# mpi4py/mpi4py-fft

Measured on AMD Instinct MI355X. Metric: pfft_3d_c2c_1024cubed_fp64_gflops, higher is better.
Workload: dtype f64; 1 GPU; PFFT 3D c2c 1024^3 complex128 forward+backward per step

## Files before the change

mpi4py-fft_amd/csrc/fft_fused_f64.hip:

```cpp
#include "fft_fused_impl.h"

namespace gfft {

#ifdef GFFT_VARIANTS
struct Fused1024x8 {
  typedef PassCfg<double, 1024, 16, 8, false, true, PF_NT_LOAD | PF_SYS_STORE | PF_NATURAL, MODE_C2C, false, 16, 16, 4> RowsToRing;
  typedef PassCfg<double, 1024, 16, 8, false, true, PF_NT_STORE | PF_SYS_LOAD | PF_NATURAL, MODE_C2C, false, 16, 16, 4> RowsFromRing;
  typedef PassCfg<double, 1024, 16, 8, true, true, PF_NT_LOAD | PF_C2C_ONLY | PF_SYS_STORE | PF_NATURAL, MODE_C2C, false, 16, 16, 4> ColsToRing;
  typedef PassCfg<double, 1024, 16, 8, true, true, PF_NT_STORE | PF_C2C_ONLY | PF_SYS_LOAD | PF_NATURAL, MODE_C2C, false, 16, 16, 4> ColsFromRing;
  typedef PassCfg<double, 1024, 16, 8, true, true, PF_NT_LOAD | PF_TRANSPOSE_STORE | PF_SYS_STORE | PF_NATURAL, MODE_C2C, true, 16, 16, 4> FourStepFirst;
  typedef PassCfg<double, 1024, 16, 8, true, true, PF_NT_LOAD | PF_SYS_STORE | PF_NATURAL, MODE_C2C, true, 16, 16, 4> FourStepFirstNat;
  typedef PassCfg<double, 1024, 16, 8, false, true, PF_NT_STORE | PF_TRANSPOSE_STORE | PF_SYS_LOAD | PF_NATURAL, MODE_C2C, false, 16, 16, 4> RowsFromRingT;
};
struct Fused1024x8R32 {
  typedef PassCfg<double, 1024, 32, 8, false, true, PF_NT_LOAD | PF_SYS_STORE | PF_NATURAL, MODE_C2C, false, 32, 32> RowsToRing;
  typedef PassCfg<double, 1024, 32, 8, false, true, PF_NT_STORE | PF_SYS_LOAD | PF_NATURAL, MODE_C2C, false, 32, 32> RowsFromRing;
  typedef PassCfg<double, 1024, 32, 8, true, true, PF_NT_LOAD | PF_C2C_ONLY | PF_SYS_STORE | PF_NATURAL, MODE_C2C, false, 32, 32> ColsToRing;
  typedef PassCfg<double, 1024, 32, 8, true, true, PF_NT_STORE | PF_C2C_ONLY | PF_SYS_LOAD | PF_NATURAL, MODE_C2C, false, 32, 32> ColsFromRing;
  typedef PassCfg<double, 1024, 32, 8, true, true, PF_NT_LOAD | PF_TRANSPOSE_STORE | PF_SYS_STORE | PF_NATURAL, MODE_C2C, true, 32, 32> FourStepFirst;
  typedef PassCfg<double, 1024, 32, 8, true, true, PF_NT_LOAD | PF_SYS_STORE | PF_NATURAL, MODE_C2C, true, 32, 32> FourStepFirstNat;
  typedef PassCfg<double, 1024, 32, 8, false, true, PF_NT_STORE | PF_TRANSPOSE_STORE | PF_SYS_LOAD | PF_NATURAL, MODE_C2C, false, 32, 32> RowsFromRingT;
};
#endif

// ... 48 lines not shown
#else
  (void)fuse2_option;
#endif
  if (n_a == n_b && (n_a == 960 || n_a == 896)) {
    if (!g_fuse2_mixv || !cr) return nullptr;
    return n_a == 960 ? fused_pair<Fused960::ColsToRing, Fused960::RowsFromRing>() : fused_pair<Fused896::ColsToRing, Fused896::RowsFromRing>();
  }
  if (n_a == 512 && n_b == 512 && g_fuse2_n512 == 2 && (cr || crb))
    return crb ? fused_pair<Fused512T32::ColsToRingB, Fused512T32::RowsFromRing>() : fused_pair<Fused512T32::ColsToRing, Fused512T32::RowsFromRing>();
  if (n_a != n_b) {
    if (!g_fuse2_mixed || !(cr || crb)) return nullptr;
    if (n_a == 512 && n_b == 1024)
      return crb ? fused_pair<Fused512T32::ColsToRingB, Fused1024R32::RowsFromRing>() : fused_pair<Fused512T32::ColsToRing, Fused1024R32::RowsFromRing>();
    if (n_a == 1024 && n_b == 512)
      return crb ? fused_pair<Fused1024R32::ColsToRingB, Fused512T32::RowsFromRing>() : fused_pair<Fused1024R32::ColsToRing, Fused512T32::RowsFromRing>();
    return nullptr;
  }
  if (n_a != 512 && n_a != 1024) return nullptr;
  if (n_a == 512 && (!g_fuse2_n512 || !(cr || crb || kind == FUSED_PLANES_2D || kind == FUSED_PLANES_2D_B))) return nullptr;
  if (kind == FUSED_PLANES_2D_B)
    return n_a == 512 ? fused_pair<Fused512R32::RowsToRing, Fused512R32::ColsFromRingB>() : fused_pair<Fused1024R32::RowsToRing, Fused1024R32::ColsFromRingB>();
  if (crb)
    return n_a == 512 ? fused_pair<Fused512R32::ColsToRingB, Fused512R32::RowsFromRing>() : fused_pair<Fused1024R32::ColsToRingB, Fused1024R32::RowsFromRing>();
  return n_a == 512 ? pair_of_kind<Fused512R32>(kind) : pair_of_kind<Fused1024R32>(kind);
}

const FusedPair *fused2_select(int precision, int kind, int fuse2_option, int n_a, int n_b) {
  const bool f32 = precision == 4;
  if (fused_kind_real(kind)) return f32 ? fused2_select_real_f32(kind, n_a, n_b) : fused2_select_real_f64(kind, n_a, n_b);
  return f32 ? fused2_select_f32(kind, n_a, n_b) : fused2_select_f64(kind, fuse2_option, n_a, n_b);
}

}
```

mpi4py-fft_amd/csrc/fft_fused_impl.h:

```cpp
#pragma once
#include "fft_pow2_impl.h"

namespace gfft {

template <typename real, int N> struct FusedCfgs;

template <typename A, typename B>
const FusedPair *fused_pair() {
  static const FusedPair p = {&A::ntiles, &B::ntiles, &launch_fused2<A, B>};
  return &p;
}

template <typename C>
static const FusedPair *pair_of_kind(int kind) {
  switch (kind) {
    case FUSED_PLANES_2D:
    case FUSED_ROWS_COLS: return fused_pair<typename C::RowsToRing, typename C::ColsFromRing>();
    case FUSED_COLS_ROWS: return fused_pair<typename C::ColsToRing, typename C::RowsFromRing>();
    case FUSED_FOURSTEP: return fused_pair<typename C::FourStepFirst, typename C::ColsFromRing>();
    case FUSED_FOURSTEP_ROWS: return fused_pair<typename C::FourStepFirstNat, typename C::RowsFromRingT>();
  }
  return nullptr;
}

const FusedPair *fused2_select_f32(int kind, int n_a, int n_b);
const FusedPair *fused2_select_real_f64(int kind, int n_a, int n_b);
const FusedPair *fused2_select_real_f32(int kind, int n_a, int n_b);

}
```

mpi4py-fft_amd/csrc/fft_pow2_impl.h:

```cpp
#pragma once
#include "gfft_internal.h"
#include "pass_io.h"

namespace gfft {

template <typename real> struct K {
  static constexpr real SQ = (real)0.70710678118654752440084436210485;
  static constexpr real C1 = (real)0.92387953251128675612818318939679;
  static constexpr real S1 = (real)0.38268343236508977172845998403040;
};

template <typename real, int S> __device__ __forceinline__ void dft2(cx<real> *v) {
  cx<real> a = v[0], b = v[S];
  v[0] = a + b;
  v[S] = a - b;
}

template <typename real> __device__ __forceinline__ void bf4(cx<real> &a0, cx<real> &a1, cx<real> &a2, cx<real> &a3) {
  cx<real> t0 = a0 + a2, t1 = a0 - a2, t2 = a1 + a3, t3 = mul_mi(a1 - a3);
  a0 = t0 + t2;
  a1 = t1 + t3;
  a2 = t0 - t2;
  a3 = t1 - t3;
}
// ... 1026 lines not shown
          }
        }
      }
    }
  }
  __syncthreads();
}

#ifdef GFFT_FUSE2_TRACE
#define GFFT_TRACE_SLOTS 96
#define GFFT_TRACE_STAMP(i)                                                                                    \
  if (it < GFFT_TRACE_SLOTS && wave_of_thread0()) {                                                              \
    if (threadIdx.x == 0) trace[((size_t)blockIdx.x * GFFT_TRACE_SLOTS + it) * 16 + (i)] = wall_clock64();      \
  }
#else
#define GFFT_TRACE_STAMP(i)
#endif

template <typename A, typename B> constexpr int fused2_per_cu() {
  constexpr size_t lds = A::lds > B::lds ? A::lds : B::lds;
  constexpr int budget = (A::regs_per_thread >= 64 || B::regs_per_thread >= 64) ? 256 : 128;
  return (2 * A::threads / 256 * budget <= 512 && 2 * lds + 1024 <= 160 * 1024) ? 2 : 1;
}
template <typename A, typename B>
__global__ void __launch_bounds__(A::threads, (fused2_per_cu<A, B>() * A::threads / 256))
fft_fused2_kernel(const PassDesc *__restrict__ descs, FusedDesc f, double scale_a, double scale_b, const void *__restrict__ in,
                  void *__restrict__ ring, void *__restrict__ out) {
  static_assert(A::threads == B::threads, "both passes of a fused pair run on one workgroup shape");
  const PassDesc &dA = descs[0], &dB = descs[1];
  extern __shared__ __attribute__((aligned(16))) unsigned char smem[];
  __shared__ unsigned tk[4];
  unsigned *done_a = f.ctr + 16, *done_b = f.ctr + 16 + f.planes;
  const unsigned grp = (unsigned)f.group;
  const unsigned ta = (unsigned)f.tiles_a / grp, tb = (unsigned)f.tiles_b / grp, per_pair = ta + tb;
  const unsigned head = (unsigned)f.lag * ta, pairs = (unsigned)(f.planes - f.lag);
  const unsigned total = (unsigned)f.planes * per_pair;
#ifdef GFFT_FUSE2_TRACE
  unsigned long long *trace = reinterpret_cast<unsigned long long *>(f.ctr + ((16 + 2 * (size_t)f.planes + 63) & ~(size_t)63));
  unsigned it = 0;
#endif
  if (wave_of_thread0()) {
    if (threadIdx.x == 0) tk[0] = atomicAdd(&f.ctr[0], 1u);
  }
  int owed = -1;
  auto settle = [&]() {
    if (owed >= 0) {
      __builtin_amdgcn_s_waitcnt(0);
      __syncthreads();
      if (wave_of_thread0()) {
        if (threadIdx.x == 0) __hip_atomic_fetch_add(&done_a[owed], 1u, __ATOMIC_RELAXED, __HIP_MEMORY_SCOPE_AGENT);
      }
      owed = -1;
    }
  };
  auto await = [&](const unsigned *flag, unsigned want) {
    if (owed >= 0) {
      if (wave_of_thread0()) {
        if (threadIdx.x == 0) tk[2] = __hip_atomic_load(flag, __ATOMIC_RELAXED, __HIP_MEMORY_SCOPE_AGENT) >= want ? 1u : 0u;
      }
// ... 7 lines not shown
#ifdef GFFT_FUSE2_TRACE
  auto hook = [&]() {
    settle();
    __builtin_amdgcn_s_waitcnt(0);
    GFFT_TRACE_STAMP(2)
  };
  for (it = 0;; ++it) {
#else
  auto &hook = settle;
  for (unsigned it = 0;; ++it) {
#endif
#ifdef GFFT_FUSE2_TRACE
    if (wave_of_thread0()) {
      if (threadIdx.x == 0) gfft_trace_slot = it < GFFT_TRACE_SLOTS ? trace + ((size_t)blockIdx.x * GFFT_TRACE_SLOTS + it) * 16 : nullptr;
    }
#endif
    __syncthreads();
    const unsigned k = __builtin_amdgcn_readfirstlane(tk[it & 1]);
    if (k >= total) break;
    GFFT_TRACE_STAMP(0)
    if (wave_of_thread0()) {
      if (threadIdx.x == 0) tk[(it + 1) & 1] = atomicAdd(&f.ctr[0], 1u);
    }
    bool is_a;
    unsigned p, t;
    if (k < head) {
      is_a = true; p = k / ta; t = k - p * ta;
    } else {
      const unsigned k2 = k - head;
      if (k2 < pairs * per_pair) {
        const unsigned j = k2 / per_pair, r = k2 - j * per_pair;
        if (r < tb) { is_a = false; p = j; t = r; } else { is_a = true; p = j + (unsigned)f.lag; t = r - tb; }
      } else {
        const unsigned k3 = k2 - pairs * per_pair, j = k3 / tb;
        is_a = false; p = pairs + j; t = k3 - j * tb;
      }
    }
    char *slot = static_cast<char *>(ring) + (size_t)(p % (unsigned)f.ring) * f.slot_bytes;
    if (f.debug == 2) continue;
#ifdef GFFT_FUSE2_TRACE
    if (it < GFFT_TRACE_SLOTS && wave_of_thread0()) {
      if (threadIdx.x == 0) trace[((size_t)blockIdx.x * GFFT_TRACE_SLOTS + it) * 16 + 7] = ((unsigned long long)k << 1) | (is_a ? 1u : 0u);
    }
#endif
    if (is_a) {
      if (p >= (unsigned)f.ring) await(&done_b[p - f.ring], tb);
      else if (f.defer == 2) settle();
      GFFT_TRACE_STAMP(1)
      if (f.debug != 3 && f.debug != 5)
        for (unsigned g = 0; g < grp; ++g)
          A::tile(dA, static_cast<const char *>(in) + (size_t)p * f.a_in_plane, slot, smem, t * grp + g, scale_a, hook);
      GFFT_TRACE_STAMP(3)
      owed = (int)p;
      if (!f.defer) settle();
      GFFT_TRACE_STAMP(4)
    } else {
      await(&done_a[p], ta);
      GFFT_TRACE_STAMP(1)
      if (f.debug != 3 && f.debug != 4)
        for (unsigned g = 0; g < grp; ++g)
          B::tile(dB, slot, static_cast<char *>(out) + (size_t)p * f.b_out_plane, smem, t * grp + g, scale_b, hook);
      GFFT_TRACE_STAMP(3)
      __syncthreads();
      if (wave_of_thread0()) {
        if (threadIdx.x == 0) __hip_atomic_fetch_add(&done_b[p], 1u, __ATOMIC_RELAXED, __HIP_MEMORY_SCOPE_AGENT);
      }
      GFFT_TRACE_STAMP(4)
    }
  }
  settle();
}


template <typename A, typename B>
hipError_t launch_fused2(const PassDesc &dA, const PassDesc &dB, const PassDesc *dev_descs, const FusedDesc &f, const void *in,
                         void *ring, void *out, hipStream_t s) {
  constexpr size_t lds = A::lds > B::lds ? A::lds : B::lds;
  static_assert(lds <= 160 * 1024, "LDS budget");
  if (f.lag < 1 || f.ring <= f.lag || f.planes < 1 || f.tiles_a != (int)A::ntiles(dA) || f.tiles_b != (int)B::ntiles(dB) ||
      f.group < 1 || f.tiles_a % f.group || f.tiles_b % f.group)
    return hipErrorInvalidValue;
  auto kern = fft_fused2_kernel<A, B>;
  static bool attr_set[kMaxDevices] = {};
  static int cus_of[kMaxDevices] = {};
  const int dev = current_device();
  if (!attr_set[dev] && lds > 64 * 1024) {
    hipError_t e = hipFuncSetAttribute(reinterpret_cast<const void *>(kern), hipFuncAttributeMaxDynamicSharedMemorySize, (int)lds);
    if (e != hipSuccess) return e;
    attr_set[dev] = true;
  }
  if (!cus_of[dev]) {
    int n = 0;
    if (hipDeviceGetAttribute(&n, hipDeviceAttributeMultiprocessorCount, dev) != hipSuccess || n < 1) { (void)hipGetLastError(); n = 256; }
    cus_of[dev] = n;
  }
  const int cus = cus_of[dev];
  hipError_t e = hipMemsetAsync(f.ctr, 0, (size_t)(16 + 2 * f.planes) * sizeof(unsigned), s);
  if (e != hipSuccess) return e;
  constexpr int per_cu = fused2_per_cu<A, B>();
  hipLaunchKernelGGL(kern, dim3(cus * per_cu), dim3(A::threads), lds, s, dev_descs, f, dA.scale, dB.scale, in, ring, out);
  return hipGetLastError();
}


template <typename real, int N, int R, int T, bool COLS, bool SPLIT, int MINW, int FLAGS, int MODE, bool BIGTW, int... RADS>
// ... 134 lines not shown
```

mpi4py-fft_amd/csrc/gfft_internal.h:

```cpp
#pragma once
#include <hip/hip_runtime.h>
#include <stdint.h>
#include <string>

namespace gfft {

int fail(int code, const std::string &msg);
int hip_fail(hipError_t e, const char *what);
int check_device();
int scratch_get(hipStream_t s, size_t bytes, void **out);
#define HIP_TRY(expr)                                        \
  do {                                                       \
    hipError_t _e = (expr);                                  \
    if (_e != hipSuccess) return gfft::hip_fail(_e, #expr);  \
  } while (0)

constexpr int kMaxDevices = 64;
inline int current_device() {
  int d = 0;
  if (hipGetDevice(&d) != hipSuccess) { (void)hipGetLastError(); d = 0; }
  return (d < 0 || d >= kMaxDevices) ? 0 : d;
}

template <typename T> struct cx { T x, y; };

template <typename T> __device__ __forceinline__ cx<T> operator+(cx<T> a, cx<T> b) { return {a.x + b.x, a.y + b.y}; }
// ... 87 lines not shown

inline bool strided_lines_whole(const PassDesc &d, int esz) {
  auto ok = [&](int64_t s) { return (s * esz) % 128 == 0; };
  if (!ok(d.in_es) || !ok(d.out_es)) return false;
  const int64_t rows = d.mid * d.inner > 0 ? d.batch / (d.mid * d.inner) : 1;
  if (d.mid > 1 && !d.flat && (!ok(d.in_ms) || !ok(d.out_ms))) return false;
  if (rows > 1 && (!ok(d.in_os) || !ok(d.out_os))) return false;
  if ((d.in_lgp && !ok(d.in_jump)) || (d.out_lgp && !ok(d.out_jump))) return false;
  return true;
}

bool pow2_supported_f64(int n);
bool pow2_supported_f32(int n);
hipError_t launch_pow2_f64(const PassDesc &d, bool cols, int variant, const void *in, void *out, hipStream_t s);
hipError_t launch_pow2_f32(const PassDesc &d, bool cols, int variant, const void *in, void *out, hipStream_t s);
bool pow2_r2r_supported(int n);
hipError_t launch_pow2_r2r_f64(const PassDesc &d, bool cols, const void *in, void *out, hipStream_t s);
hipError_t launch_pow2_r2r_f32(const PassDesc &d, bool cols, const void *in, void *out, hipStream_t s);
int pow2_grid_cap();
struct FusedDesc {
  int planes, tiles_a, tiles_b, ring, lag;
  int defer;
  int group;
  int64_t a_in_plane, b_out_plane;
  int64_t slot_bytes;
  unsigned debug;
  unsigned wait_ticks;
  unsigned plan_id;
  unsigned *host_flag;
  unsigned *ctr;
};
enum FusedKind { FUSED_ROWS_COLS = 0, FUSED_COLS_ROWS = 1, FUSED_FOURSTEP = 2, FUSED_PLANES_2D = 3, FUSED_FOURSTEP_ROWS = 4,
                 FUSED_R2C_PLANES = 5, FUSED_COLS_C2R = 6,
                 FUSED_PLANES_2D_B = 7, FUSED_PLANES_CR_B = 8,
                 FUSED_R2C_PLANES_B = 9, FUSED_COLS_C2R_B = 10 };
struct FusedKindInfo { const char *pass_name, *describe_name; bool real; };
inline constexpr FusedKindInfo kFusedKinds[] = {
  {"fused rows+cols", "rows -> strided", false},
  {"fused cols+rows", "strided -> rows", false},
  {"fused four-step", "four-step", false},
  {"fused 2-D rows+cols", "2-D planes: rows -> strided", false},
  {"fused four-step (rows)", "four-step: strided -> rows, transposed on store", false},
  {"fused r2c-rows+cols", "r2c rows -> strided", true},
  {"fused cols+c2r-rows", "strided -> c2r rows", true},
  {"fused 2-D rows+cols(blocks)", "2-D planes: rows -> strided into blocks", false},
  {"fused 2-D cols(blocks)+rows", "2-D planes: strided from blocks -> rows", false},
  {"fused 2-D r2c-rows+cols(blocks)", "2-D planes: r2c rows -> strided into blocks", true},
  {"fused 2-D cols(blocks)+c2r-rows", "2-D planes: strided from blocks -> c2r rows", true},
};
static_assert(sizeof kFusedKinds / sizeof kFusedKinds[0] == FUSED_COLS_C2R_B + 1, "one row per FusedKind");
inline bool fused_kind_real(int kind) { return kFusedKinds[kind].real; }
extern int g_fuse2_n512;
extern int g_fuse2_mixed;
extern int g_fuse2_f32_n512;
extern int g_fuse2_mixv;
extern int g_c2r_2048;
struct FusedPair {
  unsigned (*tiles_a)(const PassDesc &), (*tiles_b)(const PassDesc &);
  hipError_t (*launch)(const PassDesc &dA, const PassDesc &dB, const PassDesc *dev_descs, const FusedDesc &f, const void *in,
                       void *ring, void *out, hipStream_t s);
};
const FusedPair *fused2_select(int precision, int kind, int fuse2_option, int n_a, int n_b);

bool real_half_supported(int n_complex);
hipError_t launch_real_half_f64(const PassDesc &d, int variant, const void *in, void *out, hipStream_t s);
hipError_t launch_real_half_f32(const PassDesc &d, int variant, const void *in, void *out, hipStream_t s);
bool real_half_mix_supported(int n_complex);
hipError_t launch_real_half_mix_f64(const PassDesc &d, const void *in, void *out, hipStream_t s);
hipError_t launch_real_half_mix_f32(const PassDesc &d, const void *in, void *out, hipStream_t s);
bool mix3_supported(int n);
hipError_t launch_mix3_f64(const PassDesc &d, bool cols, const void *in, void *out, hipStream_t s);
hipError_t launch_mix3_f32(const PassDesc &d, bool cols, const void *in, void *out, hipStream_t s);
bool mixv_supported(int n);
hipError_t launch_mixv_f64(const PassDesc &d, bool cols, int variant, const void *in, void *out, hipStream_t s);
hipError_t launch_mixv_f32(const PassDesc &d, bool cols, int variant, const void *in, void *out, hipStream_t s);
hipError_t launch_real_half_mixv_f64(const PassDesc &d, const void *in, void *out, hipStream_t s);
hipError_t launch_real_half_mixv_f32(const PassDesc &d, const void *in, void *out, hipStream_t s);
bool mix5_supported(int n);
hipError_t launch_mix5_f64(const PassDesc &d, bool cols, const void *in, void *out, hipStream_t s);
hipError_t launch_mix5_f32(const PassDesc &d, bool cols, const void *in, void *out, hipStream_t s);

bool plane2d_supported(int n, int precision);
int plane2d_pitch(int n);
// ... 19 lines not shown
```

mpi4py-fft_amd/csrc/plan.cpp:

```cpp
#include "../../include/gfft.h"
#include "gfft_internal.h"

#include <atomic>
#include <cmath>
#include <cstdio>
#include <cstdlib>
#include <cstring>
#include <map>
#include <tuple>
#include <mutex>
#include <string>
#include <thread>
#include <vector>

using namespace gfft;

namespace {

thread_local std::string g_last_error;
bool g_device_checked = false;

}

namespace gfft {
// ... 23 lines not shown
}

namespace {

struct Options {
  int grid_cap = 0;
  int variant_rows = 0;
  int variant_cols = 0;
  int force_generic = 0;
  int xcd_swizzle = -1;
  int tile_order = -1;
  int profile = 0;
  int fused3 = 1;
  int debug_flat = 0;
  int flat_out = 1;
  int mixv_variant = 0;
  int mixv = 1;
  int wtile = 1;
  int plane2d = 1;
  int fuse2 = 1;
  int fuse2_ring = 0, fuse2_lag = 0;
  int fuse2_kinds = 2046;
  int fuse2_f32 = 1;
  int fuse2_wait_ms = 2000;
  int debug_tile_lg = 0, debug_tile_side = 0, debug_tile_stride = 0;
  int64_t fused3_min_bytes = 32 << 20;
  int debug_tw_index = 1, debug_tw_exp = 0, debug_tw_len = 0;
  int debug_r2r_index = 1, debug_r2r_exp = 0, debug_r2r_post = 0;
  Options() {
    if (const char *s = getenv("GFFT_GRID_CAP")) grid_cap = atoi(s);
    if (const char *s = getenv("GFFT_VARIANT_ROWS")) variant_rows = atoi(s);
    if (const char *s = getenv("GFFT_VARIANT_COLS")) variant_cols = atoi(s);
    if (const char *s = getenv("GFFT_FORCE_GENERIC")) force_generic = atoi(s);
    if (const char *s = getenv("GFFT_FUSED3")) fused3 = atoi(s);
    if (const char *s = getenv("GFFT_XCD_SWIZZLE")) xcd_swizzle = atoi(s);
    if (const char *s = getenv("GFFT_FUSE2")) fuse2 = atoi(s);
    if (const char *s = getenv("GFFT_FUSE2_RING")) fuse2_ring = atoi(s);
    if (const char *s = getenv("GFFT_FUSE2_LAG")) fuse2_lag = atoi(s);
    if (const char *s = getenv("GFFT_FUSE2_KINDS")) fuse2_kinds = atoi(s);
    if (const char *s = getenv("GFFT_FUSE2_WAIT_MS")) fuse2_wait_ms = atoi(s);
  }
};
Options &opts() {
  static Options o;
  return o;
}

int dev_prec(int precision) { return precision + (current_device() << 8); }
std::mutex g_tw_mutex;
std::map<std::tuple<int64_t, int, int>, void *> g_tw_cache;
struct BigTw { void *hi, *lo; int L; };
std::map<std::pair<int64_t, int>, BigTw> g_bigtw_cache;

int upload_twiddles(int64_t n, int64_t step, int64_t count, int precision, void **out, int64_t wrong_index = -1, double wrong_by = 0) {
  const long double w = -2.0L * 3.14159265358979323846264338327950288L / (long double)n;
  std::vector<unsigned char> host((size_t)count * 2 * precision);
  for (int64_t j = 0; j < count; ++j) {
    const int64_t k = (j * step) % n;
    long double c, s;
    {
      const long double a = w * (long double)k;
      c = cosl(a);
      s = sinl(a);
// ... 67 lines not shown
  bool regk = false, cols = false;
  int src = BUF_IN, dst = BUF_OUT;
  bool carries_scale = false;
  bool logical_first = false;
  PointDesc pt{};
  double extra_scale = 1.0;
  bool has_full = false;
  PassDesc full{};
  int64_t data_inner = 0;
  int blocks[2] = {1, 1};
  int64_t bstride[2] = {0, 0};
  PassDesc d2{};
  FusedDesc fused{};
  int fused_kind = 0;
  const FusedPair *pair = nullptr;
  PassDesc *dev_descs = nullptr;
  int alt_first = -1;
  int alt_buf = -1;
  size_t alt_bytes = 0;
  double bytes2 = 0;
};

bool make_fused2(gfft_plan_s *pl, int kind, const Pass &a, const Pass &b, const PassDesc &dA, const PassDesc &dB, int planes,
                 int64_t a_in_plane, int64_t b_out_plane, int64_t slot_bytes, Pass *out);

bool is_pow2(int64_t n) { return n > 0 && (n & (n - 1)) == 0; }

static int pow2_rows_nt(int64_t n, int precision) {
  if (!is_pow2(n) || n < 16 || n > 4096) return 0;
  if (n <= 32) return 4;
  if (n == 64) return 8;
  if (n == 128) return 16;
  if (n == 256) return precision == 8 ? 32 : 16;
  if (n <= 1024) return 64;
  return (int)(n / 16);
}

bool regk_ok(int64_t n, int precision) {
  if (opts().force_generic) return false;
  if (n > 4096) return false;
  if (mix3_supported((int)n) || mix5_supported((int)n)) return true;
  return precision == 8 ? pow2_supported_f64((int)n) : pow2_supported_f32((int)n);
}

bool regk_c2c_ok(int64_t n, int precision, int mode) {
  (void)precision;
  return !opts().force_generic && opts().mixv && mode == MODE_C2C && n <= 4096 && mixv_supported((int)n);
// ... 257 lines not shown
    if (hipGetDeviceProperties(&prop, dev) == hipSuccess) {
      if (!strncmp(prop.gcnArchName, "gfx942", 6) || !strncmp(prop.gcnArchName, "gfx950", 6)) arch_ok[dev] = 1;
    } else {
      (void)hipGetLastError();
    }
  }
  return arch_ok[dev] > 0;
}

struct PairChoice {
  const FusedPair *pair = nullptr;
  int ring = 0, lag = 0;
};
PairChoice fused2_pair(int precision, int kind, int n_a, int n_b, int64_t slot_bytes, int planes) {
  PairChoice c;
  if (!fused2_arch_ok()) return c;
  if (!opts().fuse2 || !((opts().fuse2_kinds >> kind) & 1)) return c;
  if (precision == GFFT_F32 && (!opts().fuse2_f32 || (fused_kind_real(kind) && opts().fuse2_f32 < 2))) return c;
  if (!fused2_ring(precision, n_a, n_b, slot_bytes, planes, &c.ring, &c.lag)) return c;
  c.pair = fused2_select(precision, kind, opts().fuse2, n_a, n_b);
  return c;
}

bool make_fused2(gfft_plan_s *pl, int kind, const Pass &a, const Pass &b, const PassDesc &dA, const PassDesc &dB, int planes,
                 int64_t a_in_plane, int64_t b_out_plane, int64_t slot_bytes, Pass *out) {
  const PairChoice c = fused2_pair(pl->precision, kind, dA.n, dB.n, slot_bytes, planes);
  if (!c.pair) return false;
  const int ta = (int)c.pair->tiles_a(dA), tb = (int)c.pair->tiles_b(dB);
  if (ta < 1 || tb < 1) return false;
  if (slot_bytes >= ((int64_t)1 << 31) || (double)planes * (ta + tb) >= 1.0e9) return false;
  Pass f = a;
  f.kind = PK_FUSED2;
  f.fused_kind = kind;
  f.pair = c.pair;
  f.d = dA;
  f.d2 = dB;
  f.src = a.src;
  f.dst = b.dst;
  f.carries_scale = false;
  f.fused.planes = planes;
  f.fused.tiles_a = ta;
  f.fused.tiles_b = tb;
  f.fused.ring = c.ring;
  f.fused.lag = c.lag;
  f.fused.defer = 0;
  f.fused.group = 1;
  f.fused.a_in_plane = a_in_plane;
  f.fused.b_out_plane = b_out_plane;
  f.fused.slot_bytes = (int64_t)align256((size_t)slot_bytes);
  f.fused.ctr = nullptr;
  f.fused.wait_ticks = 0;
  f.fused.plan_id = pl->id;
  f.fused.host_flag = nullptr;
  f.fused.debug = 0;
  for (const Pass *q : {&a, &b})
    for (int side : {q->src, q->dst})
      if (side >= BUF_WS && side != BUF_RING) f.alt_buf = side;

  size_t ctr_bytes = align256((size_t)(16 + 2 * planes) * sizeof(unsigned));
#ifdef GFFT_FUSE2_TRACE
  ctr_bytes += 256 + (size_t)1024 * 96 * 16 * sizeof(unsigned long long);
#endif
  const PassDesc both[2] = {f.d, f.d2};
  void *dev = nullptr;
  if (hipMalloc(&dev, sizeof both) != hipSuccess) { (void)hipGetLastError(); return false; }
  if (hipMemcpy(dev, both, sizeof both, hipMemcpyHostToDevice) != hipSuccess) { (void)hipGetLastError(); (void)hipFree(dev); return false; }
  pl->device_allocs.push_back(dev);
  f.dev_descs = static_cast<PassDesc *>(dev);
  need(pl, BUF_RING, (size_t)c.ring * (size_t)f.fused.slot_bytes + ctr_bytes);
  f.alt_first = (int)pl->alt.size();
  pl->alt.push_back(a);
  pl->alt.push_back(b);
  *out = f;
  return true;
}

struct Line {
  int64_t outer, inner, n, nin, nout;
  int mode;
  bool inverse;
  int src, dst;
};

int plan_line(gfft_plan_s *pl, const Line &L, bool top);

PassDesc natural_desc(const Line &L) {
  PassDesc d{};
  d.n = (int)L.n;
  d.mode = L.mode;
  d.conj_in = L.inverse ? 1 : 0;
  d.conj_out = (L.inverse && L.mode != MODE_C2R) ? 1 : 0;
  d.batch = L.outer * L.inner;
// ... 689 lines not shown
    seq.push_back(axis0_flat(BUF_WS, BUF_OUT));
  } else if (!inverse && !cols_first) {
    seq.push_back(rows(real ? MODE_R2C : MODE_C2C, false, true, BUF_IN, BUF_WS));
    seq.push_back(axis0(BUF_WS, BUF_WS));
    seq.push_back(axis1(true, false, BUF_WS, BUF_OUT));
  } else {
    seq.push_back(axis1(false, true, BUF_IN, BUF_WS));
    seq.push_back(axis0(BUF_WS, BUF_WS));
    seq.push_back(rows(real ? MODE_C2R : MODE_C2C, true, false, BUF_WS, BUF_OUT));
  }
  for (Pass &p : seq) {
    int rc = get_twiddles(p.d.n, prec, &p.d.tw);
    if (rc) return rc;
    const bool half = p.d.mode == MODE_R2C_H || p.d.mode == MODE_C2R_H;
    if (half && (rc = get_twiddles(2 * (int64_t)p.d.n, prec, &p.d.rtw))) return rc;
    const double lines = p.data_inner ? (double)p.d.batch / (double)p.d.inner * (double)p.data_inner : (double)p.d.batch;
    const double n = half ? 2.0 * p.d.n : p.d.n;
    pl->flops += (p.d.mode == MODE_C2C ? 1.0 : 0.5) * 5.0 * n * std::log2(n) * lines;
    pl->bytes += fused3_pass_bytes(p, prec, nc_full);
    pl->passes.push_back(p);
  }
  auto fuse = [&](size_t i, int kind, const PassDesc &dA, const PassDesc &dB, int64_t planes, int64_t a_in_plane, int64_t b_out_plane, int64_t slot_bytes) {
    Pass f;
    if (!make_fused2(pl, kind, pl->passes[i], pl->passes[i + 1], dA, dB, (int)planes, a_in_plane, b_out_plane, slot_bytes, &f)) return;
    f.bytes2 = fused3_pass_bytes(pl->passes[i], prec, nc_full) + fused3_pass_bytes(pl->passes[i + 1], prec, nc_full);
    pl->passes[i] = f;
    pl->passes.erase(pl->passes.begin() + i + 1);
  };
  if (!real && !tr && !flat_out && Pu == nc && pl->passes.size() >= 3) {
    const size_t base = pl->passes.size() - 3;
    const Pass &p1 = pl->passes[base], &p2 = pl->passes[base + 1], &p3 = pl->passes[base + 2];
    if (!inverse && !cols_first) {
      PassDesc dA = p1.d, dB = p2.d;
      dA.batch = n0; dA.inner = 1; dA.in_is = 0; dA.out_is = 0; dA.out_os = P;
      dB.batch = Pu; dB.in_os = 0; dB.out_os = 0; dB.in_es = P;
      fuse(base, FUSED_ROWS_COLS, dA, dB, n1, n2 * esz, w_i1 * esz, n0 * P * esz);
    } else {
      PassDesc dA = p2.d, dB = p3.d;
      dA.batch = Pu; dA.in_os = 0; dA.out_os = 0; dA.out_es = P;
      dB.batch = n0; dB.inner = 1; dB.in_is = 0; dB.out_is = 0; dB.in_os = P; dB.out_os = n1 * n2;
      int64_t a_plane = w_i1 * esz;
      if (wtile) {
        dA.mid = Pu / TWc; dA.inner = TWc;
        dA.in_ms = wtS; dA.in_is = 1; dA.in_ilg = 0; dA.in_iS = 0;
        dA.out_ms = TWc;     dA.out_is = 1; dA.out_ilg = 0; dA.out_iS = 0;
        dB.in_tlg = 0; dB.in_tS = 0;
        a_plane = TWc * esz;
// ... 281 lines not shown
}

int gfft_device_name(int device, char *buf, size_t len) {
  hipDeviceProp_t prop;
  HIP_TRY(hipGetDeviceProperties(&prop, device));
  snprintf(buf, len, "%s (%s, %d CUs)", prop.name, prop.gcnArchName, prop.multiProcessorCount);
  return GFFT_OK;
}

int gfft_set_option(const char *key, int value) {
  if (!key) return fail(GFFT_ERR_INVALID, "null option name");
  if (!strcmp(key, "grid_cap")) opts().grid_cap = value;
  else if (!strcmp(key, "variant_rows")) opts().variant_rows = value;
  else if (!strcmp(key, "variant_cols")) opts().variant_cols = value;
  else if (!strcmp(key, "force_generic")) opts().force_generic = value;
  else if (!strcmp(key, "copy_nt")) gfft::g_copy_nt = value;
  else if (!strcmp(key, "fused3")) opts().fused3 = value;
  else if (!strcmp(key, "plane2d")) opts().plane2d = value;
  else if (!strcmp(key, "fuse2")) opts().fuse2 = value;
  else if (!strcmp(key, "fuse2_ring")) opts().fuse2_ring = value;
  else if (!strcmp(key, "fuse2_lag")) opts().fuse2_lag = value;
  else if (!strcmp(key, "fuse2_kinds")) opts().fuse2_kinds = value;
  else if (!strcmp(key, "fuse2_wait_ms")) opts().fuse2_wait_ms = value;
  else if (!strcmp(key, "fuse2_f32")) opts().fuse2_f32 = value;
  else if (!strcmp(key, "fuse2_n512")) gfft::g_fuse2_n512 = value;
  else if (!strcmp(key, "c2r_2048")) gfft::g_c2r_2048 = value;
  else if (!strcmp(key, "fuse2_mixv")) gfft::g_fuse2_mixv = value;
  else if (!strcmp(key, "fuse2_mixed")) gfft::g_fuse2_mixed = value;
  else if (!strcmp(key, "fuse2_f32_n512")) gfft::g_fuse2_f32_n512 = value;
  else if (!strcmp(key, "debug_flat")) opts().debug_flat = value;
  else if (!strcmp(key, "flat_out")) opts().flat_out = value;
  else if (!strcmp(key, "wtile")) opts().wtile = value;
  else if (!strcmp(key, "mixv")) opts().mixv = value;
  else if (!strcmp(key, "mixv_variant")) opts().mixv_variant = value;
  else if (!strcmp(key, "debug_tile_lg")) opts().debug_tile_lg = value;
  else if (!strcmp(key, "debug_tile_side")) opts().debug_tile_side = value;
  else if (!strcmp(key, "debug_tile_stride")) opts().debug_tile_stride = value;
  else if (!strcmp(key, "profile")) opts().profile = value;
  else if (!strcmp(key, "debug_tw_index")) opts().debug_tw_index = value;
  else if (!strcmp(key, "debug_tw_exp")) opts().debug_tw_exp = value;
  else if (!strcmp(key, "debug_tw_len")) opts().debug_tw_len = value;
  else if (!strcmp(key, "debug_r2r_index")) opts().debug_r2r_index = value;
  else if (!strcmp(key, "debug_r2r_exp")) opts().debug_r2r_exp = value;
  else if (!strcmp(key, "debug_r2r_post")) opts().debug_r2r_post = value;
  else if (!strcmp(key, "xcd_swizzle")) opts().xcd_swizzle = value;
  else if (!strcmp(key, "tile_order")) opts().tile_order = value;
// ... 287 lines not shown
        const Pass &q = pl->alt[p.alt_first + k];
        PassDesc dq = q.d;
        const bool sc = k == 1 && p.carries_scale;
        if (sc) dq.scale = scale;
        HIP_TRY(run_pass(pl, q, dq, bufs[q.src], bufs[q.dst], sc ? scale : 1.0, s));
      }
      HIP_TRY(mark());
      continue;
    }
    if (p.kind == PK_FUSED2) {
      PassDesc d2 = p.d2;
      if (p.carries_scale) d2.scale = scale;
      FusedDesc f = p.fused;
      char *ring = static_cast<char *>(bufs[BUF_RING]);
      f.ctr = reinterpret_cast<unsigned *>(ring + (size_t)f.ring * (size_t)f.slot_bytes);
      {
        AsyncErrors &ae = async_errors();
        f.host_flag = (ae.flag && pl->async_slot >= 0) ? ae.flag + pl->async_slot : nullptr;
        const int ms = opts().fuse2_wait_ms;
        f.wait_ticks = ms <= 0 ? 0u : (ms > 40000 ? 4000000000u : (unsigned)ms * 100000u);
      }
      static const int debug = getenv("GFFT_FUSE2_DEBUG") ? atoi(getenv("GFFT_FUSE2_DEBUG")) : 0;
      if (debug) { f.wait_ticks = 100000u; f.host_flag = nullptr; f.debug = (unsigned)debug; }
      HIP_TRY(p.pair->launch(d, d2, p.dev_descs, f, bufs[p.src], ring, bufs[p.dst], s));
      if (debug) {
        HIP_TRY(hipStreamSynchronize(s));
        std::vector<unsigned> h(16 + 2 * (size_t)f.planes);
        HIP_TRY(hipMemcpy(h.data(), f.ctr, h.size() * sizeof(unsigned), hipMemcpyDeviceToHost));
        unsigned long long sa = 0, sb = 0;
        for (int i = 0; i < f.planes; ++i) { sa += h[16 + i]; sb += h[16 + f.planes + i]; }
        fprintf(stderr, "[gfft fuse2] kind %d planes %d tiles %d+%d ring %d lag %d: tickets %u, waits given up %u, A tiles %llu, B tiles %llu\n",
                p.fused_kind, f.planes, f.tiles_a, f.tiles_b, f.ring, f.lag, h[0], h[1], sa, sb);
#ifdef GFFT_FUSE2_TRACE
        if (const char *path = getenv("GFFT_FUSE2_TRACE_FILE")) {
          std::vector<unsigned long long> tr((size_t)1024 * 96 * 16);
          const size_t off = ((16 + 2 * (size_t)f.planes + 63) & ~(size_t)63) * sizeof(unsigned);
          HIP_TRY(hipMemcpy(tr.data(), reinterpret_cast<char *>(f.ctr) + off, tr.size() * sizeof(tr[0]), hipMemcpyDeviceToHost));
          if (FILE *fp = fopen(path, "wb")) { fwrite(tr.data(), sizeof(tr[0]), tr.size(), fp); fclose(fp); }
        }
#endif
      }
      HIP_TRY(mark());
      continue;
    }
    if (p.carries_scale) d.scale = scale;
    HIP_TRY(run_pass(pl, p, d, bufs[p.src], bufs[p.dst], p.carries_scale ? scale : 1.0, s));
    HIP_TRY(mark());
// ... 428 lines not shown
  d.ub_tlg = lg;
  for (int b = 0; b < 8; ++b) d.ub_base[b] = b < nblocks ? d.ub_rows * (int64_t)d.ub_start[b] : 0;
  return GFFT_OK;
}

int gfft_scratch_release(void) { return scratch_pool().release(true); }

int gfft_async_error(void) { return poll_async_error(nullptr); }
int gfft_plan_status(gfft_plan pl) {
  if (!pl) return fail(GFFT_ERR_INVALID, "null plan");
  return poll_async_error(pl);
}

int gfft_plan_destroy(gfft_plan pl) {
  if (!pl) return GFFT_OK;
  delete pl;
  if (--g_live_plans == 0) (void)scratch_pool().release(false);
  return GFFT_OK;
}

int gfft_plan_describe(gfft_plan pl, char *buf, size_t len) {
  if (!pl || !buf || !len) return fail(GFFT_ERR_INVALID, "null argument");
  std::string s;
  char line[256];
  const char *kn = pl->kind == GFFT_C2C_FORWARD ? "c2c-forward" : pl->kind == GFFT_C2C_BACKWARD ? "c2c-backward"
                   : pl->kind == GFFT_R2C ? "r2c" : "c2r";
  char sched[96] = "";
  if (pl->fused3 && pl->ws_tile) snprintf(sched, sizeof sched, " [3-D schedule: tile-major workspace, tiles of %d columns]", pl->ws_tile);
  else if (pl->fused3) snprintf(sched, sizeof sched, " [3-D schedule: padded-pitch workspace, rows %lld entries apart]", (long long)pl->ws_pitch);
  snprintf(line, sizeof line, "gfft plan: %s %s, %d dims, %zu passes%s\n", kn, pl->precision == 8 ? "f64" : "f32",
           pl->ndims, pl->passes.size(), sched);
  s += line;
  static const char *bufn[] = {"IN", "OUT", "WS", "FS", "AUX", "RING", "FS2"};
  for (const Pass &p : pl->passes) {
    if (p.kind == PK_FUSED2) {
      const char *fk = kFusedKinds[p.fused_kind].describe_name;
      if (pl->fused_off)
        snprintf(line, sizeof line, "  pair (%s) n=%d then n=%d as two stand-alone passes (a fused launch gave up a wait)%s  %s -> %s\n",
                 fk, p.d.n, p.d2.n, p.carries_scale ? " [scale]" : "", bufn[p.src], bufn[p.dst]);
      else
      snprintf(line, sizeof line, "  fused pair (%s) n=%d then n=%d: %d planes, %d + %d tiles per plane, ring of %d slots x %lld KiB, one persistent launch%s  %s -> %s\n",
               fk, p.d.n, p.d2.n, p.fused.planes, p.fused.tiles_a, p.fused.tiles_b, p.fused.ring,
               (long long)(p.fused.slot_bytes >> 10), p.carries_scale ? " [scale]" : "", bufn[p.src], bufn[p.dst]);
      s += line;
      continue;
    }
    if (p.kind == PK_PLANE2D) {
      snprintf(line, sizeof line, "  planes on chip: rows n=%d then columns n=%d of %d planes held in LDS, one launch%s  %s -> %s\n", p.d.n, p.d2.n,
               p.fused.planes, p.carries_scale ? " [scale]" : "", bufn[p.src], bufn[p.dst]);
      s += line;
      continue;
    }
    if (p.kind != PK_FFT) {
      static const char *kinds[] = {"", "embed (chirp/zero-pad into AUX)", "multiply by B = FFT(chirp)", "extract (chirp, scale)"};
      snprintf(line, sizeof line, "  %s n=%lld Lw=%lld  %s -> %s\n", kinds[p.kind], (long long)p.pt.n,
               (long long)p.pt.Lw, bufn[p.src], bufn[p.dst]);
      s += line;
      continue;
    }
    snprintf(line, sizeof line, "  n=%d batch=%lld (mid=%lld inner=%lld) es_in=%lld es_out=%lld kernel=%s%s%s  %s -> %s\n",
             p.d.n, (long long)p.d.batch, (long long)p.d.mid, (long long)p.d.inner, (long long)p.d.in_es,
             (long long)p.d.out_es,
             (p.d.mode == MODE_R2C_H || p.d.mode == MODE_C2R_H) ? "regs-rows packed-real (n = complex length)"
             : p.regk ? (p.cols ? "regs-cols" : "regs-rows") : "generic",
             p.d.tw_hi ? " [four-step 1/2, fused twiddle]" : "", p.carries_scale ? " [scale]" : "",
             bufn[p.src], bufn[p.dst]);
// ... 145 lines not shown
```

Before: 10570 GFLOP/s.

## Add paired-plane ticket order for fused 1024 cols-rows persistent kernel

Adds a second ticket-to-work mapping for the persistent fused two-pass kernel. Planes are interleaved in pairs spaced d apart, and the ring size and lag are re-planned so the ring gap constraints still hold. It is enabled by default for the f64 1024x1024 cols-rows pair under the 3-D schedule. The goal is to change the order in which stage-A and stage-B tiles are processed, which affects locality and how long workers wait on plane dependencies. In exchange it may enlarge the ring buffer (up to 256 MiB) and adds extra index arithmetic per ticket.

```diff
diff --git a/mpi4py-fft_amd/csrc/fft_fused_f64.hip b/mpi4py-fft_amd/csrc/fft_fused_f64.hip
--- a/mpi4py-fft_amd/csrc/fft_fused_f64.hip
+++ b/mpi4py-fft_amd/csrc/fft_fused_f64.hip
@@ -94,6 +94,7 @@
     return n_a == 512 ? fused_pair<Fused512R32::RowsToRing, Fused512R32::ColsFromRingB>() : fused_pair<Fused1024R32::RowsToRing, Fused1024R32::ColsFromRingB>();
   if (crb)
     return n_a == 512 ? fused_pair<Fused512R32::ColsToRingB, Fused512R32::RowsFromRing>() : fused_pair<Fused1024R32::ColsToRingB, Fused1024R32::RowsFromRing>();
+  if (cr && n_a == 1024) return fused_pair<Fused1024R32::ColsToRing, Fused1024R32::RowsFromRing, true>();
   return n_a == 512 ? pair_of_kind<Fused512R32>(kind) : pair_of_kind<Fused1024R32>(kind);
 }
 
diff --git a/mpi4py-fft_amd/csrc/fft_fused_impl.h b/mpi4py-fft_amd/csrc/fft_fused_impl.h
--- a/mpi4py-fft_amd/csrc/fft_fused_impl.h
+++ b/mpi4py-fft_amd/csrc/fft_fused_impl.h
@@ -5,10 +5,15 @@
 
 template <typename real, int N> struct FusedCfgs;
 
-template <typename A, typename B>
+template <typename A, typename B, bool WITH_PAIR_ORDER = false>
 const FusedPair *fused_pair() {
-  static const FusedPair p = {&A::ntiles, &B::ntiles, &launch_fused2<A, B>};
-  return &p;
+  if constexpr (WITH_PAIR_ORDER) {
+    static const FusedPair p = {&A::ntiles, &B::ntiles, &launch_fused2<A, B>, &launch_fused2<A, B, true>};
+    return &p;
+  } else {
+    static const FusedPair p = {&A::ntiles, &B::ntiles, &launch_fused2<A, B>, nullptr};
+    return &p;
+  }
 }
 
 template <typename C>
diff --git a/mpi4py-fft_amd/csrc/fft_pow2_impl.h b/mpi4py-fft_amd/csrc/fft_pow2_impl.h
--- a/mpi4py-fft_amd/csrc/fft_pow2_impl.h
+++ b/mpi4py-fft_amd/csrc/fft_pow2_impl.h
@@ -1072,7 +1072,7 @@
   constexpr int budget = (A::regs_per_thread >= 64 || B::regs_per_thread >= 64) ? 256 : 128;
   return (2 * A::threads / 256 * budget <= 512 && 2 * lds + 1024 <= 160 * 1024) ? 2 : 1;
 }
-template <typename A, typename B>
+template <typename A, typename B, bool PAIR_ORDER = false>
 __global__ void __launch_bounds__(A::threads, (fused2_per_cu<A, B>() * A::threads / 256))
 fft_fused2_kernel(const PassDesc *__restrict__ descs, FusedDesc f, double scale_a, double scale_b, const void *__restrict__ in,
                   void *__restrict__ ring, void *__restrict__ out) {
@@ -1082,9 +1082,8 @@
   __shared__ unsigned tk[4];
   unsigned *done_a = f.ctr + 16, *done_b = f.ctr + 16 + f.planes;
   const unsigned grp = (unsigned)f.group;
-  const unsigned ta = (unsigned)f.tiles_a / grp, tb = (unsigned)f.tiles_b / grp, per_pair = ta + tb;
-  const unsigned head = (unsigned)f.lag * ta, pairs = (unsigned)(f.planes - f.lag);
-  const unsigned total = (unsigned)f.planes * per_pair;
+  const unsigned ta = (unsigned)f.tiles_a / grp, tb = (unsigned)f.tiles_b / grp;
+  const unsigned total = (unsigned)f.planes * (ta + tb);
 #ifdef GFFT_FUSE2_TRACE
   unsigned long long *trace = reinterpret_cast<unsigned long long *>(f.ctr + ((16 + 2 * (size_t)f.planes + 63) & ~(size_t)63));
   unsigned it = 0;
@@ -1138,20 +1137,13 @@
     if (wave_of_thread0()) {
       if (threadIdx.x == 0) tk[(it + 1) & 1] = atomicAdd(&f.ctr[0], 1u);
     }
-    bool is_a;
-    unsigned p, t;
-    if (k < head) {
-      is_a = true; p = k / ta; t = k - p * ta;
-    } else {
-      const unsigned k2 = k - head;
-      if (k2 < pairs * per_pair) {
-        const unsigned j = k2 / per_pair, r = k2 - j * per_pair;
-        if (r < tb) { is_a = false; p = j; t = r; } else { is_a = true; p = j + (unsigned)f.lag; t = r - tb; }
-      } else {
-        const unsigned k3 = k2 - pairs * per_pair, j = k3 / tb;
-        is_a = false; p = pairs + j; t = k3 - j * tb;
-      }
-    }
+    FusedTicket tkt;
+    if constexpr (PAIR_ORDER)
+      tkt = fused_ticket(k, ta, tb, (unsigned)f.planes, (unsigned)f.lag >> 1, fused_order_upair((unsigned)f.planes, (unsigned)f.d), (unsigned)f.d);
+    else
+      tkt = fused_ticket_plain(k, ta, tb, (unsigned)f.planes, (unsigned)f.lag);
+    const bool is_a = tkt.is_a;
+    const unsigned p = tkt.plane, t = tkt.tile;
     char *slot = static_cast<char *>(ring) + (size_t)(p % (unsigned)f.ring) * f.slot_bytes;
     if (f.debug == 2) continue;
 #ifdef GFFT_FUSE2_TRACE
@@ -1188,7 +1180,7 @@
 }
 
 
-template <typename A, typename B>
+template <typename A, typename B, bool PAIR_ORDER = false>
 hipError_t launch_fused2(const PassDesc &dA, const PassDesc &dB, const PassDesc *dev_descs, const FusedDesc &f, const void *in,
                          void *ring, void *out, hipStream_t s) {
   constexpr size_t lds = A::lds > B::lds ? A::lds : B::lds;
@@ -1196,7 +1188,8 @@
   if (f.lag < 1 || f.ring <= f.lag || f.planes < 1 || f.tiles_a != (int)A::ntiles(dA) || f.tiles_b != (int)B::ntiles(dB) ||
       f.group < 1 || f.tiles_a % f.group || f.tiles_b % f.group)
     return hipErrorInvalidValue;
-  auto kern = fft_fused2_kernel<A, B>;
+  if ((f.order != 0) != PAIR_ORDER || (f.order && ((f.lag & 1) || !fused_order_fits(f.planes, f.ring, f.lag / 2, f.d)))) return hipErrorInvalidValue;
+  auto kern = fft_fused2_kernel<A, B, PAIR_ORDER>;
   static bool attr_set[kMaxDevices] = {};
   static int cus_of[kMaxDevices] = {};
   const int dev = current_device();
diff --git a/mpi4py-fft_amd/csrc/fused_order.h b/mpi4py-fft_amd/csrc/fused_order.h
--- /dev/null
+++ b/mpi4py-fft_amd/csrc/fused_order.h
@@ -0,0 +1,113 @@
+#pragma once
+
+#if defined(__HIPCC__)
+#define GFFT_HD __host__ __device__ __forceinline__
+#else
+#define GFFT_HD inline
+#endif
+
+namespace gfft {
+
+struct FusedTicket {
+  bool is_a;
+  unsigned plane, tile;
+};
+
+GFFT_HD FusedTicket fused_ticket_plain(unsigned k, unsigned ta, unsigned tb, unsigned planes, unsigned lag) {
+  FusedTicket t;
+  const unsigned per_pair = ta + tb, head = lag * ta, pairs = planes - lag;
+  if (k < head) {
+    t.is_a = true; t.plane = k / ta; t.tile = k - t.plane * ta;
+  } else {
+    const unsigned k2 = k - head;
+    if (k2 < pairs * per_pair) {
+      const unsigned j = k2 / per_pair, r = k2 - j * per_pair;
+      if (r < tb) { t.is_a = false; t.plane = j; t.tile = r; } else { t.is_a = true; t.plane = j + lag; t.tile = r - tb; }
+    } else {
+      const unsigned k3 = k2 - pairs * per_pair, j = k3 / tb;
+      t.is_a = false; t.plane = pairs + j; t.tile = k3 - j * tb;
+    }
+  }
+  return t;
+}
+
+GFFT_HD unsigned fused_order_upair(unsigned planes, unsigned d) { return d ? (planes / (2u * d)) * d : 0u; }
+GFFT_HD unsigned fused_order_unit(unsigned p, unsigned upair, unsigned d) {
+  return p < 2u * upair ? (p / (2u * d)) * d + (p % (2u * d)) % d : p - upair;
+}
+
+GFFT_HD void fused_order_locate(unsigned x, unsigned n, unsigned v0, unsigned upair, unsigned d, unsigned &plane, unsigned &tile) {
+  const unsigned in_pairs = v0 < upair ? (upair - v0) * 2u * n : 0u;
+  if (x < in_pairs) {
+    const unsigned v = v0 + x / (2u * n), r = x % (2u * n);
+    plane = (v / d) * 2u * d + v % d + (r & 1u) * d;
+    tile = r >> 1;
+  } else {
+    x -= in_pairs;
+    plane = (v0 > upair ? v0 : upair) + upair + x / n;
+    tile = x % n;
+  }
+}
+
+GFFT_HD FusedTicket fused_ticket(unsigned k, unsigned ta, unsigned tb, unsigned planes, unsigned lead, unsigned upair, unsigned d) {
+  FusedTicket t;
+  const unsigned head = (lead + (lead < upair ? lead : upair)) * ta;
+  if (k < head) {
+    t.is_a = true;
+    fused_order_locate(k, ta, 0u, upair, d, t.plane, t.tile);
+    return t;
+  }
+  k -= head;
+  const unsigned jm = planes - upair - lead;
+  const unsigned j1 = upair > lead ? upair - lead : 0u;
+  const unsigned j2 = upair < jm ? upair : jm;
+  unsigned j0 = 0u, nj = j1, sb = 2u * tb, sa = 2u * ta;
+  if (k >= nj * (sa + sb)) {
+    k -= nj * (sa + sb);
+    j0 = j1; nj = j2 - j1; sa = ta;
+    if (k >= nj * (sa + sb)) {
+      k -= nj * (sa + sb);
+      j0 = j2; nj = jm - j2; sb = tb;
+      if (k >= nj * (sa + sb)) {
+        k -= nj * (sa + sb);
+        t.is_a = false;
+        fused_order_locate(k, tb, jm, upair, d, t.plane, t.tile);
+        return t;
+      }
+    }
+  }
+  const unsigned j = j0 + k / (sa + sb), r = k % (sa + sb);
+  t.is_a = r >= sb;
+  if (t.is_a) fused_order_locate(r - sb, ta, j + lead, upair, d, t.plane, t.tile);
+  else fused_order_locate(r, tb, j, upair, d, t.plane, t.tile);
+  return t;
+}
+
+inline int fused_order_gap(int planes, int ring, int d) {
+  const unsigned upair = fused_order_upair((unsigned)planes, (unsigned)d);
+  int gap = planes;
+  for (int p = ring; p < planes; ++p) {
+    const int g = (int)fused_order_unit((unsigned)p, upair, (unsigned)d) - (int)fused_order_unit((unsigned)(p - ring), upair, (unsigned)d);
+    if (g < gap) gap = g;
+  }
+  return gap;
+}
+inline bool fused_order_fits(int planes, int ring, int lead, int d) {
+  if (d < 1 || lead < 1 || planes < 2 * d || ring <= 2 * lead) return false;
+  const int upair = (int)fused_order_upair((unsigned)planes, (unsigned)d);
+  if (planes - upair < lead) return false;
+  return fused_order_gap(planes, ring, d) >= lead;
+}
+
+inline bool fused_order_plan(int planes, int d, int ring_max, int *ring, int *lag) {
+  const int lead = (*lag + 2) / 2, gap = (*ring + 1) / 2;
+  for (int r = *ring; r <= ring_max && planes >= 2 * r; ++r)
+    if (fused_order_fits(planes, r, lead, d) && fused_order_gap(planes, r, d) >= gap) {
+      *ring = r;
+      *lag = 2 * lead;
+      return true;
+    }
+  return false;
+}
+
+}
diff --git a/mpi4py-fft_amd/csrc/gfft_internal.h b/mpi4py-fft_amd/csrc/gfft_internal.h
--- a/mpi4py-fft_amd/csrc/gfft_internal.h
+++ b/mpi4py-fft_amd/csrc/gfft_internal.h
@@ -2,6 +2,7 @@
 #include <hip/hip_runtime.h>
 #include <stdint.h>
 #include <string>
+#include "fused_order.h"
 
 namespace gfft {
 
@@ -135,6 +136,7 @@
   int planes, tiles_a, tiles_b, ring, lag;
   int defer;
   int group;
+  int order, d;
   int64_t a_in_plane, b_out_plane;
   int64_t slot_bytes;
   unsigned debug;
@@ -172,6 +174,8 @@
   unsigned (*tiles_a)(const PassDesc &), (*tiles_b)(const PassDesc &);
   hipError_t (*launch)(const PassDesc &dA, const PassDesc &dB, const PassDesc *dev_descs, const FusedDesc &f, const void *in,
                        void *ring, void *out, hipStream_t s);
+  hipError_t (*launch_pair_order)(const PassDesc &dA, const PassDesc &dB, const PassDesc *dev_descs, const FusedDesc &f, const void *in,
+                                  void *ring, void *out, hipStream_t s);
 };
 const FusedPair *fused2_select(int precision, int kind, int fuse2_option, int n_a, int n_b);
 
diff --git a/mpi4py-fft_amd/csrc/plan.cpp b/mpi4py-fft_amd/csrc/plan.cpp
--- a/mpi4py-fft_amd/csrc/plan.cpp
+++ b/mpi4py-fft_amd/csrc/plan.cpp
@@ -69,6 +69,7 @@
   int fuse2_ring = 0, fuse2_lag = 0;
   int fuse2_kinds = 2046;
   int fuse2_f32 = 1;
+  int fuse2_order = -1, fuse2_order_d = 2;
   int fuse2_wait_ms = 2000;
   int debug_tile_lg = 0, debug_tile_side = 0, debug_tile_stride = 0;
   int64_t fused3_min_bytes = 32 << 20;
@@ -86,6 +87,8 @@
     if (const char *s = getenv("GFFT_FUSE2_LAG")) fuse2_lag = atoi(s);
     if (const char *s = getenv("GFFT_FUSE2_KINDS")) fuse2_kinds = atoi(s);
     if (const char *s = getenv("GFFT_FUSE2_WAIT_MS")) fuse2_wait_ms = atoi(s);
+    if (const char *s = getenv("GFFT_FUSE2_ORDER")) fuse2_order = atoi(s);
+    if (const char *s = getenv("GFFT_FUSE2_ORDER_D")) fuse2_order_d = atoi(s);
   }
 };
 Options &opts() {
@@ -199,7 +202,7 @@
 };
 
 bool make_fused2(gfft_plan_s *pl, int kind, const Pass &a, const Pass &b, const PassDesc &dA, const PassDesc &dB, int planes,
-                 int64_t a_in_plane, int64_t b_out_plane, int64_t slot_bytes, Pass *out);
+                 int64_t a_in_plane, int64_t b_out_plane, int64_t slot_bytes, Pass *out, bool schedule3d = false);
 
 bool is_pow2(int64_t n) { return n > 0 && (n & (n - 1)) == 0; }
 
@@ -503,8 +506,10 @@
   return c;
 }
 
+constexpr int kHeadlinePairOrder = 1;
+
 bool make_fused2(gfft_plan_s *pl, int kind, const Pass &a, const Pass &b, const PassDesc &dA, const PassDesc &dB, int planes,
-                 int64_t a_in_plane, int64_t b_out_plane, int64_t slot_bytes, Pass *out) {
+                 int64_t a_in_plane, int64_t b_out_plane, int64_t slot_bytes, Pass *out, bool schedule3d) {
   const PairChoice c = fused2_pair(pl->precision, kind, dA.n, dB.n, slot_bytes, planes);
   if (!c.pair) return false;
   const int ta = (int)c.pair->tiles_a(dA), tb = (int)c.pair->tiles_b(dB);
@@ -524,6 +529,18 @@
   f.fused.tiles_b = tb;
   f.fused.ring = c.ring;
   f.fused.lag = c.lag;
+  f.fused.order = 0;
+  f.fused.d = 0;
+  {
+    const bool headline = schedule3d && kind == FUSED_COLS_ROWS && pl->precision == GFFT_F64 && dA.n == 1024 && dB.n == 1024;
+    const int want = opts().fuse2_order < 0 ? (headline ? kHeadlinePairOrder : 0) : opts().fuse2_order;
+    const int64_t sb = (int64_t)align256((size_t)slot_bytes);
+    const int ring_max = opts().fuse2_ring > 0 ? c.ring : std::max<int>(c.ring, (int)(((int64_t)256 << 20) / (sb > 0 ? sb : 1)));
+    if (want == 1 && c.pair->launch_pair_order && fused_order_plan(planes, opts().fuse2_order_d, ring_max, &f.fused.ring, &f.fused.lag)) {
+      f.fused.order = 1;
+      f.fused.d = opts().fuse2_order_d;
+    }
+  }
   f.fused.defer = 0;
   f.fused.group = 1;
   f.fused.a_in_plane = a_in_plane;
@@ -548,7 +565,7 @@
   if (hipMemcpy(dev, both, sizeof both, hipMemcpyHostToDevice) != hipSuccess) { (void)hipGetLastError(); (void)hipFree(dev); return false; }
   pl->device_allocs.push_back(dev);
   f.dev_descs = static_cast<PassDesc *>(dev);
-  need(pl, BUF_RING, (size_t)c.ring * (size_t)f.fused.slot_bytes + ctr_bytes);
+  need(pl, BUF_RING, (size_t)f.fused.ring * (size_t)f.fused.slot_bytes + ctr_bytes);
   f.alt_first = (int)pl->alt.size();
   pl->alt.push_back(a);
   pl->alt.push_back(b);
@@ -1284,7 +1301,7 @@
   }
   auto fuse = [&](size_t i, int kind, const PassDesc &dA, const PassDesc &dB, int64_t planes, int64_t a_in_plane, int64_t b_out_plane, int64_t slot_bytes) {
     Pass f;
-    if (!make_fused2(pl, kind, pl->passes[i], pl->passes[i + 1], dA, dB, (int)planes, a_in_plane, b_out_plane, slot_bytes, &f)) return;
+    if (!make_fused2(pl, kind, pl->passes[i], pl->passes[i + 1], dA, dB, (int)planes, a_in_plane, b_out_plane, slot_bytes, &f, true)) return;
     f.bytes2 = fused3_pass_bytes(pl->passes[i], prec, nc_full) + fused3_pass_bytes(pl->passes[i + 1], prec, nc_full);
     pl->passes[i] = f;
     pl->passes.erase(pl->passes.begin() + i + 1);
@@ -1612,6 +1629,8 @@
   else if (!strcmp(key, "fuse2_lag")) opts().fuse2_lag = value;
   else if (!strcmp(key, "fuse2_kinds")) opts().fuse2_kinds = value;
   else if (!strcmp(key, "fuse2_wait_ms")) opts().fuse2_wait_ms = value;
+  else if (!strcmp(key, "fuse2_order")) opts().fuse2_order = value;
+  else if (!strcmp(key, "fuse2_order_d")) opts().fuse2_order_d = value;
   else if (!strcmp(key, "fuse2_f32")) opts().fuse2_f32 = value;
   else if (!strcmp(key, "fuse2_n512")) gfft::g_fuse2_n512 = value;
   else if (!strcmp(key, "c2r_2048")) gfft::g_c2r_2048 = value;
@@ -1945,7 +1964,7 @@
       }
       static const int debug = getenv("GFFT_FUSE2_DEBUG") ? atoi(getenv("GFFT_FUSE2_DEBUG")) : 0;
       if (debug) { f.wait_ticks = 100000u; f.host_flag = nullptr; f.debug = (unsigned)debug; }
-      HIP_TRY(p.pair->launch(d, d2, p.dev_descs, f, bufs[p.src], ring, bufs[p.dst], s));
+      HIP_TRY((f.order ? p.pair->launch_pair_order : p.pair->launch)(d, d2, p.dev_descs, f, bufs[p.src], ring, bufs[p.dst], s));
       if (debug) {
         HIP_TRY(hipStreamSynchronize(s));
         std::vector<unsigned> h(16 + 2 * (size_t)f.planes);
@@ -2420,7 +2439,7 @@
 int gfft_plan_describe(gfft_plan pl, char *buf, size_t len) {
   if (!pl || !buf || !len) return fail(GFFT_ERR_INVALID, "null argument");
   std::string s;
-  char line[256];
+  char line[384];
   const char *kn = pl->kind == GFFT_C2C_FORWARD ? "c2c-forward" : pl->kind == GFFT_C2C_BACKWARD ? "c2c-backward"
                    : pl->kind == GFFT_R2C ? "r2c" : "c2r";
   char sched[96] = "";
@@ -2433,13 +2452,15 @@
   for (const Pass &p : pl->passes) {
     if (p.kind == PK_FUSED2) {
       const char *fk = kFusedKinds[p.fused_kind].describe_name;
+      char ord[48] = "plain";
+      if (p.fused.order) snprintf(ord, sizeof ord, "pairs of planes d = %d", p.fused.d);
       if (pl->fused_off)
         snprintf(line, sizeof line, "  pair (%s) n=%d then n=%d as two stand-alone passes (a fused launch gave up a wait)%s  %s -> %s\n",
                  fk, p.d.n, p.d2.n, p.carries_scale ? " [scale]" : "", bufn[p.src], bufn[p.dst]);
       else
-      snprintf(line, sizeof line, "  fused pair (%s) n=%d then n=%d: %d planes, %d + %d tiles per plane, ring of %d slots x %lld KiB, one persistent launch%s  %s -> %s\n",
+      snprintf(line, sizeof line, "  fused pair (%s) n=%d then n=%d: %d planes, %d + %d tiles per plane, ring of %d slots x %lld KiB, lead %d planes, ticket order %d (%s), one persistent launch%s  %s -> %s\n",
                fk, p.d.n, p.d2.n, p.fused.planes, p.fused.tiles_a, p.fused.tiles_b, p.fused.ring,
-               (long long)(p.fused.slot_bytes >> 10), p.carries_scale ? " [scale]" : "", bufn[p.src], bufn[p.dst]);
+               (long long)(p.fused.slot_bytes >> 10), p.fused.lag, p.fused.order, ord, p.carries_scale ? " [scale]" : "", bufn[p.src], bufn[p.dst]);
       s += line;
       continue;
     }
```

New measurement: 10550 GFLOP/s. About the same (-0.2%).
